# cg-tuwien/ppsurf

Measured on AMD Instinct MI355X. Metric: occupancy query-points/sec @ res=257, 50NN, higher is better.
Workload: dtype f16x3

## Files before the change

### ppsurf_amd/csrc/pps_common.h

```cpp
#pragma once
#include <hip/hip_runtime.h>
#include <stdint.h>

typedef float f32x4 __attribute__((ext_vector_type(4)));

#define PPS_WAVE 64
#define PPS_OK 0
#define PPS_ERR_ARG 1
#define PPS_ERR_LAUNCH 2

#define PPS_SG_MFMA 0x008
#define PPS_SG_DSREAD 0x100
#define PPS_SG_VALU 0x002

namespace pps {

__device__ __forceinline__ int lane_id() { return threadIdx.x & 63; }

template <int CTRL>
__device__ __forceinline__ float dpp_mov(float v) {
    return __builtin_bit_cast(float, __builtin_amdgcn_update_dpp(0, __builtin_bit_cast(int, v), CTRL, 0xf, 0xf, true));
}
__device__ __forceinline__ float row16_max(float v) {
    v = fmaxf(v, dpp_mov<0xB1>(v));
// ... 123 lines not shown
            for (int r = 0; r < 4; ++r) {
                acc0[r] = fmaxf(acc0[r], 0.f);
                acc1[r] = fmaxf(acc1[r], 0.f);
            }
        }
        out[ob] = acc0;
        out[ob + 1] = acc1;
    }
}

typedef _Float16 half8 __attribute__((ext_vector_type(8)));
typedef unsigned u32x4 __attribute__((ext_vector_type(4)));
struct HiLo { half8 hi, lo; };

__device__ __forceinline__ HiLo split_f16(const f32x4& x0, const f32x4& x1) {
    u32x4 hp, lp;
    const float v[8] = {x0.x, x0.y, x0.z, x0.w, x1.x, x1.y, x1.z, x1.w};
#pragma unroll
    for (int p = 0; p < 4; ++p) {
        const unsigned h = __builtin_bit_cast(unsigned, __builtin_amdgcn_cvt_pkrtz(v[2 * p], v[2 * p + 1]));
        unsigned l;
        asm("v_fma_mixlo_f16 %0, %1, -1.0, %2 op_sel_hi:[1,0,0]" : "=v"(l) : "v"(h), "v"(v[2 * p]));
        asm("v_fma_mixhi_f16 %0, %1, -1.0, %2 op_sel:[1,0,0] op_sel_hi:[1,0,0]" : "+v"(l) : "v"(h), "v"(v[2 * p + 1]));
        hp[p] = h;
        lp[p] = l;
    }
    return HiLo{__builtin_bit_cast(half8, hp), __builtin_bit_cast(half8, lp)};
}
#define PPS_F16_MAX 65504.f
__device__ __forceinline__ void range_track(float& amax, const f32x4& a, const f32x4& b) {
    asm volatile("v_max3_f32 %0, %0, |%1|, |%2|\n\tv_max3_f32 %0, %0, |%3|, |%4|" : "+v"(amax) : "v"(a.x), "v"(a.y), "v"(a.z), "v"(a.w));
    asm volatile("v_max3_f32 %0, %0, |%1|, |%2|\n\tv_max3_f32 %0, %0, |%3|, |%4|" : "+v"(amax) : "v"(b.x), "v"(b.y), "v"(b.z), "v"(b.w));
}
__device__ __forceinline__ HiLo split_f16_r(float& amax, const f32x4& x0, const f32x4& x1) {
    range_track(amax, x0, x1);
    return split_f16(x0, x1);
}
__device__ __forceinline__ void range_commit(float amax, int* flag) {
    if (flag != nullptr && !(amax <= PPS_F16_MAX)) atomicOr(flag, 1);
}
__device__ __forceinline__ bool gate_closed(const int* gate) { return gate != nullptr && __builtin_nontemporal_load(gate) == 0; }

__device__ __forceinline__ void join_f16(const HiLo& x, f32x4& y0, f32x4& y1) {
    const u32x4 hp = __builtin_bit_cast(u32x4, x.hi), lp = __builtin_bit_cast(u32x4, x.lo);
#pragma unroll
    for (int p = 0; p < 4; ++p) {
        float a, b;
        asm("v_fma_mix_f32 %0, %1, 1.0, %2 op_sel_hi:[1,0,1]" : "=v"(a) : "v"(hp[p]), "v"(lp[p]));
        asm("v_fma_mix_f32 %0, %1, 1.0, %2 op_sel:[1,0,1] op_sel_hi:[1,0,1]" : "=v"(b) : "v"(hp[p]), "v"(lp[p]));
        if (p < 2) { y0[2 * p] = a; y0[2 * p + 1] = b; } else { y1[2 * (p - 2)] = a; y1[2 * (p - 2) + 1] = b; }
    }
}

template <int KB, int NOB, int ACT, bool FENCE = true, bool INIT = false, class Sink, class Hook>
__device__ __forceinline__ void dense_blocks_f16x3_hook(const HiLo (&in)[KB], const half8* __restrict__ w, const f32x4* __restrict__ bias, int lane,
                                                        Sink&& sink, Hook&& hook, const f32x4* init = nullptr) {
    static_assert(NOB % 2 == 0, "output blocks are processed in pairs");
    const int g = lane >> 4;
#pragma unroll
    for (int ob = 0; ob < NOB; ob += 2) {
        f32x4 m0 = INIT ? init[ob] : bias[(ob) * 4 + g], m1 = INIT ? init[ob + 1] : bias[(ob + 1) * 4 + g];
        f32x4 c0 = {0.f, 0.f, 0.f, 0.f}, c1 = {0.f, 0.f, 0.f, 0.f};
        const half8* w0 = w + ((ob) * KB) * 128 + lane;
        const half8* w1 = w + ((ob + 1) * KB) * 128 + lane;
        half8 ph0 = w0[0], pl0 = w0[64], ph1 = w1[0], pl1 = w1[64];
#pragma unroll
        for (int kb = 0; kb < KB; ++kb) {
            const half8 ah0 = ph0, al0 = pl0, ah1 = ph1, al1 = pl1;
            if (kb + 1 < KB) {
                ph0 = w0[(kb + 1) * 128]; pl0 = w0[(kb + 1) * 128 + 64];
                ph1 = w1[(kb + 1) * 128]; pl1 = w1[(kb + 1) * 128 + 64];
            }
            m0 = __builtin_amdgcn_mfma_f32_16x16x32_f16(ah0, in[kb].hi, m0, 0, 0, 0);
            m1 = __builtin_amdgcn_mfma_f32_16x16x32_f16(ah1, in[kb].hi, m1, 0, 0, 0);
            c0 = __builtin_amdgcn_mfma_f32_16x16x32_f16(ah0, in[kb].lo, c0, 0, 0, 0);
            c1 = __builtin_amdgcn_mfma_f32_16x16x32_f16(ah1, in[kb].lo, c1, 0, 0, 0);
            c0 = __builtin_amdgcn_mfma_f32_16x16x32_f16(al0, in[kb].hi, c0, 0, 0, 0);
            c1 = __builtin_amdgcn_mfma_f32_16x16x32_f16(al1, in[kb].hi, c1, 0, 0, 0);
            hook(ob, kb);
            if (FENCE) {
                __builtin_amdgcn_sched_group_barrier(PPS_SG_DSREAD, 4, 0);
                __builtin_amdgcn_sched_group_barrier(PPS_SG_MFMA, 6, 0);
                __builtin_amdgcn_sched_barrier(0);
            }
        }
        f32x4 o0 = m0 + c0, o1 = m1 + c1;
        if (ACT == 1) {
#pragma unroll
            for (int r = 0; r < 4; ++r) { o0[r] = fmaxf(o0[r], 0.f); o1[r] = fmaxf(o1[r], 0.f); }
        }
        sink(ob >> 1, o0, o1);
    }
}
template <int KB, int NOB, int ACT, bool FENCE = true, bool INIT = false, class Sink>
__device__ __forceinline__ void dense_blocks_f16x3(const HiLo (&in)[KB], const half8* __restrict__ w, const f32x4* __restrict__ bias, int lane,
                                                   Sink&& sink, const f32x4* init = nullptr) {
    dense_blocks_f16x3_hook<KB, NOB, ACT, FENCE, INIT>(in, w, bias, lane, sink, [](int, int) {}, init);
}

template <int T, int KB, int NOB, int ACT, bool FENCE = true, class Sink>
__device__ __forceinline__ void dense_blocks_f16x3_tiles(const HiLo (&in)[T][KB], const half8* __restrict__ w, const f32x4* __restrict__ bias, int lane,
                                                         Sink&& sink) {
    static_assert(NOB % 2 == 0, "output blocks are processed in pairs");
    const int g = lane >> 4;
#pragma unroll
    for (int ob = 0; ob < NOB; ob += 2) {
        f32x4 m0[T], m1[T], c0[T], c1[T];
        const f32x4 b0 = bias[(ob) * 4 + g], b1 = bias[(ob + 1) * 4 + g];
#pragma unroll
        for (int t = 0; t < T; ++t) { m0[t] = b0; m1[t] = b1; c0[t] = f32x4{0.f, 0.f, 0.f, 0.f}; c1[t] = c0[t]; }
        const half8* w0 = w + ((ob) * KB) * 128 + lane;
        const half8* w1 = w + ((ob + 1) * KB) * 128 + lane;
        half8 ph0 = w0[0], pl0 = w0[64], ph1 = w1[0], pl1 = w1[64];
#pragma unroll
        for (int kb = 0; kb < KB; ++kb) {
            const half8 ah0 = ph0, al0 = pl0, ah1 = ph1, al1 = pl1;
            if (kb + 1 < KB) {
                ph0 = w0[(kb + 1) * 128]; pl0 = w0[(kb + 1) * 128 + 64];
                ph1 = w1[(kb + 1) * 128]; pl1 = w1[(kb + 1) * 128 + 64];
            }
#pragma unroll
            for (int t = 0; t < T; ++t) {
                m0[t] = __builtin_amdgcn_mfma_f32_16x16x32_f16(ah0, in[t][kb].hi, m0[t], 0, 0, 0);
                m1[t] = __builtin_amdgcn_mfma_f32_16x16x32_f16(ah1, in[t][kb].hi, m1[t], 0, 0, 0);
                c0[t] = __builtin_amdgcn_mfma_f32_16x16x32_f16(ah0, in[t][kb].lo, c0[t], 0, 0, 0);
                c1[t] = __builtin_amdgcn_mfma_f32_16x16x32_f16(ah1, in[t][kb].lo, c1[t], 0, 0, 0);
                c0[t] = __builtin_amdgcn_mfma_f32_16x16x32_f16(al0, in[t][kb].hi, c0[t], 0, 0, 0);
                c1[t] = __builtin_amdgcn_mfma_f32_16x16x32_f16(al1, in[t][kb].hi, c1[t], 0, 0, 0);
            }
            if (FENCE) {
                __builtin_amdgcn_sched_group_barrier(PPS_SG_DSREAD, 4, 0);
                __builtin_amdgcn_sched_group_barrier(PPS_SG_MFMA, 6 * T, 0);
                __builtin_amdgcn_sched_barrier(0);
            }
        }
#pragma unroll
        for (int t = 0; t < T; ++t) {
            f32x4 o0 = m0[t] + c0[t], o1 = m1[t] + c1[t];
            if (ACT == 1) {
#pragma unroll
                for (int r = 0; r < 4; ++r) { o0[r] = fmaxf(o0[r], 0.f); o1[r] = fmaxf(o1[r], 0.f); }
            }
            sink(t, ob >> 1, o0, o1);
        }
    }
}

template <int NOB>
__device__ __forceinline__ void xyz_blocks(float coord, f32x4* acc, const float* __restrict__ wxyz, int lane) {
#pragma unroll
// ... 51 lines not shown
```

### ppsurf_amd/csrc/pps_decode.hip

```cpp
#include <cstdlib>
#include "pps_common.h"
#include "../../include/ppsurf_amd.h"

using namespace pps;

#define NT 256
#define NW (NT / 64)
#define WG_PER_CU (512 / NT)
#ifndef PPS_PRIO
#define PPS_PRIO 1
#endif
#ifndef PPS_PRIO_PN
#define PPS_PRIO_PN 1
#endif
#define CH4 2048

template <int CHUNK_F4_NEXT, int NTH = NT, class F>
__device__ __forceinline__ void stream_step(const f32x4* __restrict__ gnext, f32x4*& cur, f32x4*& nxt, F&& compute) {
    chunk_copy_async<CHUNK_F4_NEXT / NTH, NTH>(gnext, nxt);
    compute((const f32x4*)cur);
    stream_wait();
    __syncthreads();
    f32x4* t = cur; cur = nxt; nxt = t;
}
// ... 833 lines not shown
    const int lane = lane_id(), wave = threadIdx.x >> 6, n = lane & 15, g = lane >> 4;

    lds_fill(bias_l, bias + 192, 4096);
    const f32x4* bias_g = (const f32x4*)bias;
    f32x4 *cur, *nxt;
    stream_begin<CH4>(wg, cur, nxt);
    const int ntiles = (int)((Q + NW * 16 - 1) / (NW * 16));
    int first, count, stride;
    xcd_tile_range(ntiles, first, count, stride);
    for (int it = 0; it < count; ++it) {
        const TileRow q = tile_row(first + it * stride, wave, n, Q);
        HiLo u[2];
        stn_head_h(gin + q.c * 256, wg, wg + 5 * CH4, bias_g, cur, nxt, lane, amax, u);
        half8* dst = trans2h + q.c * 1024 + g;
#pragma unroll 1
        for (int c = 0; c < 32; ++c) {
            const f32x4* gn = (c + 1 < 32) ? wg + (6 + c) * CH4 : wg;
            stream_step<CH4>(gn, cur, nxt, [&](const f32x4* w) {
                dense_blocks_f16x3<2, 8, 0, false>(u, (const half8*)w, bias4 + 32 * c, lane, [&](int i, const f32x4& o0, const f32x4& o1) {
                    const int a = 2 * c + (i >> 1), kb = i & 1;
                    const HiLo v = split_f16_r(amax, o0, o1);
                    if (q.valid) {
                        half8* d = dst + (((a >> 4) * 2 + kb) * 2) * 64 + 4 * (a & 15);
                        d[0] = v.hi;
                        d[64] = v.lo;
                    }
                }); });
        }
    }
    range_commit(amax, range);
}

#define PC_W_XYZ 256
#define PC_NBIAS (576 + 256 + 4)
#define PC_WFLOATS (4096 + 8192)
#define PC_LDS_BYTES ((PC_WFLOATS + PC_W_XYZ + PC_NBIAS) * 4)

struct PhaseC {
    const f32x4 *w_c0b, *w_c2, *bias4, *u4;
    const float* xyz_l;
};
template <int NTH>
__device__ __forceinline__ PhaseC phase_c_setup(const float* __restrict__ wpack, const f32x4* __restrict__ wdense, const float* __restrict__ bias) {
    f32x4* w_l = (f32x4*)pps_smem;
    float* xyz_l = (float*)(w_l + PC_WFLOATS / 4);
    float* bias_l = xyz_l + PC_W_XYZ;
    for (int i = threadIdx.x; i < PC_WFLOATS / 4; i += NTH) w_l[i] = wdense[i];
    lds_fill(xyz_l, wpack, PC_W_XYZ);
    lds_fill(bias_l, bias, PC_NBIAS);
    const f32x4* bias4 = (const f32x4*)bias_l;
    return PhaseC{w_l, w_l + 1024, bias4, bias4 + 144, xyz_l};
}

template <bool H>
__device__ __forceinline__ void feat_rows_query(const float* __restrict__ patches, int64_t q, int P, int ntile_rows, const half8 (&th)[4][2],
                                                const half8 (&tl)[4][2], const f32x4 (&tf)[4][4], const PhaseC& pc, float s0, float& amax, int lane,
                                                float* __restrict__ xbar) {
    const int n = lane & 15, g = lane >> 4;
    const f32x4 *bias4 = pc.bias4, *u4 = pc.u4, *w_c0b = pc.w_c0b, *w_c2 = pc.w_c2;
    const float* xyz_l = pc.xyz_l;
    f32x4 acc[8];
    float mrun = -INFINITY, ssum = 0.f;
#pragma unroll
    for (int bb = 0; bb < 8; ++bb) acc[bb] = f32x4{0.f, 0.f, 0.f, 0.f};
    for (int rb = 0; rb < ntile_rows; ++rb) {
        const int rowi = rb * 16 + n;
        const bool valid = rowi < P;
        const int rowc = valid ? rowi : P - 1;
        const float coord = (g < 3) ? patches[(q * P + rowc) * 3 + g] : 0.f;
        f32x4 x0[4], y[8];
#pragma unroll
        for (int bb = 0; bb < 4; ++bb) x0[bb] = bias4[4 * bb + g];
        xyz_blocks<4>(coord, x0, xyz_l, lane);
        relu_blocks<4>(x0);
        __builtin_amdgcn_s_setprio(PPS_PRIO_PN);
        float s = 0.f;
        if (H) {
            HiLo a[2], b[2];
            a[0] = split_f16_r(amax, x0[0], x0[1]);
            a[1] = split_f16_r(amax, x0[2], x0[3]);
            dense_blocks_f16x3<2, 4, 1>(a, (const half8*)w_c0b, bias4 + 16, lane, [&](int i, const f32x4& o0, const f32x4& o1) { b[i] = split_f16_r(amax, o0, o1); });
#pragma unroll
            for (int ob = 0; ob < 4; ++ob) {
                f32x4 o = bias4[32 + 4 * ob + g], c = {0.f, 0.f, 0.f, 0.f};
#pragma unroll
                for (int kb = 0; kb < 2; ++kb) {
                    o = __builtin_amdgcn_mfma_f32_16x16x32_f16(th[ob][kb], b[kb].hi, o, 0, 0, 0);
                    c = __builtin_amdgcn_mfma_f32_16x16x32_f16(th[ob][kb], b[kb].lo, c, 0, 0, 0);
                    c = __builtin_amdgcn_mfma_f32_16x16x32_f16(tl[ob][kb], b[kb].hi, c, 0, 0, 0);
                }
                o += c;
#pragma unroll
                for (int r = 0; r < 4; ++r) x0[ob][r] = fmaxf(o[r], 0.f);
            }
            a[0] = split_f16_r(amax, x0[0], x0[1]);
            a[1] = split_f16_r(amax, x0[2], x0[3]);
            dense_blocks_f16x3<2, 8, 1>(a, (const half8*)w_c2, bias4 + 48, lane, [&](int i, const f32x4& o0, const f32x4& o1) {
                const f32x4 w0 = u4[4 * (2 * i) + g], w1 = u4[4 * (2 * i + 1) + g];
#pragma unroll
                for (int r = 0; r < 4; ++r) s += w0[r] * o0[r] + w1[r] * o1[r];
                y[2 * i] = o0;
                y[2 * i + 1] = o1;
            });
        } else {
            f32x4 x1[4];
            dense_blocks<4, 4, 1>(x0, x1, w_c0b, bias4 + 16, lane);
#pragma unroll
            for (int ob = 0; ob < 4; ++ob) {
                f32x4 o = bias4[32 + 4 * ob + g];
#pragma unroll
                for (int kb = 0; kb < 4; ++kb) {
                    o = __builtin_amdgcn_mfma_f32_16x16x4f32(tf[ob][kb].x, x1[kb].x, o, 0, 0, 0);
                    o = __builtin_amdgcn_mfma_f32_16x16x4f32(tf[ob][kb].y, x1[kb].y, o, 0, 0, 0);
                    o = __builtin_amdgcn_mfma_f32_16x16x4f32(tf[ob][kb].z, x1[kb].z, o, 0, 0, 0);
                    o = __builtin_amdgcn_mfma_f32_16x16x4f32(tf[ob][kb].w, x1[kb].w, o, 0, 0, 0);
                }
#pragma unroll
                for (int r = 0; r < 4; ++r) x0[ob][r] = fmaxf(o[r], 0.f);
            }
            dense_blocks<4, 8, 1>(x0, y, w_c2, bias4 + 48, lane);
#pragma unroll
            for (int bb = 0; bb < 8; ++bb) {
                const f32x4 w4 = u4[4 * bb + g];
#pragma unroll
                for (int r = 0; r < 4; ++r) s += w4[r] * y[bb][r];
            }
        }
        __builtin_amdgcn_s_setprio(0);
        s += __shfl_xor(s, 16);
        s += __shfl_xor(s, 32);
        s += s0;
        const float mblk = row16_max(valid ? s : -INFINITY);
        const float mnew = fmaxf(mrun, mblk);
        const float scale = __expf(mrun - mnew);
        const float en = valid ? __expf(s - mnew) : 0.f;
        mrun = mnew;
        ssum = ssum * scale + en;
#pragma unroll
        for (int bb = 0; bb < 8; ++bb)
#pragma unroll
            for (int r = 0; r < 4; ++r) acc[bb][r] = acc[bb][r] * scale + en * y[bb][r];
    }
    const float inv = 1.f / row16_sum(ssum);
    rows16_sum_transposed8(acc, lane);
    if (n < 8) ((f32x4*)(xbar + q * 128))[4 * n + g] = acc[0] * inv;
}

template <bool H>
__global__ __launch_bounds__(PNT, 2) void pointnet_feat_rows_kernel(const float* __restrict__ patches, const float* __restrict__ trans2,
                                                                    int64_t Q, int P, const float* __restrict__ wpack,
                                                                    const f32x4* __restrict__ wdense, const float* __restrict__ bias,
                                                                    float* __restrict__ xbar, int* __restrict__ flag) {
    if (!H && gate_closed(flag)) return;
    float amax = 0.f;
    const int lane = lane_id(), wave = threadIdx.x >> 6, n = lane & 15, g = lane >> 4;
    const PhaseC pc = phase_c_setup<PNT>(wpack, wdense, bias);
    __syncthreads();
    const float s0 = ((const float*)pc.bias4)[576 + 256];
    const int ntile_rows = (P + 15) / 16;

    const int ntiles = (int)((Q + PNW - 1) / PNW);
    int first, count, stride;
    xcd_tile_range(ntiles, first, count, stride);
    for (int it = 0; it < count; ++it) {
        const int64_t q = (int64_t)(first + it * stride) * PNW + wave;
        if (q >= Q) continue;
        half8 th[4][2], tl[4][2];
        f32x4 tf[4][4];
        if (H) {
            const half8* tq = (const half8*)trans2 + q * 1024 + 4 * n + g;
#pragma unroll
            for (int ob = 0; ob < 4; ++ob)
#pragma unroll
                for (int kb = 0; kb < 2; ++kb) { th[ob][kb] = tq[((ob * 2 + kb) * 2) * 64]; tl[ob][kb] = tq[((ob * 2 + kb) * 2 + 1) * 64]; }
        } else {
            const f32x4* tq = (const f32x4*)(trans2 + q * 4096);
#pragma unroll
            for (int ob = 0; ob < 4; ++ob)
#pragma unroll
                for (int kb = 0; kb < 4; ++kb) tf[ob][kb] = tq[(16 * ob + n) * 16 + 4 * kb + g];
        }
        feat_rows_query<H>(patches, q, P, ntile_rows, th, tl, tf, pc, s0, amax, lane, xbar);
    }
    if (H) range_commit(amax, flag);
}

#define PH_LDS_BYTES (2 * CH4 * 16)
__global__ __launch_bounds__(NT, 2) void pointnet_stn_head_h_kernel(const float* __restrict__ gin, int64_t Q, const f32x4* __restrict__ w16,
                                                                    const float* __restrict__ bias, half8* __restrict__ uh, int* __restrict__ range) {
    float amax = 0.f;
    const f32x4* wg = w16;
    const int lane = lane_id(), wave = threadIdx.x >> 6, n = lane & 15, g = lane >> 4;
    const f32x4* bias_g = (const f32x4*)bias;
    f32x4 *cur, *nxt;
    stream_begin<CH4>(wg, cur, nxt);
    const int ntiles = (int)((Q + NW * 16 - 1) / (NW * 16));
    int first, count, stride;
    xcd_tile_range(ntiles, first, count, stride);
    for (int it = 0; it < count; ++it) {
        const TileRow q = tile_row(first + it * stride, wave, n, Q);
        HiLo u[2];
        stn_head_h(gin + q.c * 256, wg, wg, bias_g, cur, nxt, lane, amax, u);
        if (q.valid) {
            half8* dst = uh + q.c * 16 + g;
#pragma unroll
            for (int kb = 0; kb < 2; ++kb) { dst[(2 * kb) * 4] = u[kb].hi; dst[(2 * kb + 1) * 4] = u[kb].lo; }
        }
    }
    range_commit(amax, range);
}

#define PF_NT 512
#define PF_QSTRIDE 257
#define PF_BUF (8 * PF_QSTRIDE)
#define PF_LDS_BYTES (PC_LDS_BYTES + 3 * PF_BUF * 16)
__global__ __launch_bounds__(PF_NT, 2) void pointnet_fc3_feat_rows_kernel(const float* __restrict__ patches, const half8* __restrict__ uh,
                                                                          int64_t Q, int P, const f32x4* __restrict__ wfc,
                                                                          const float* __restrict__ bias_fc, const float* __restrict__ wpack,
                                                                          const f32x4* __restrict__ wdense, const float* __restrict__ bias,
                                                                          float* __restrict__ xbar, int* __restrict__ flag) {
    float amax = 0.f;
    half8* ex = (half8*)(pps_smem + PC_LDS_BYTES);
    const int lane = lane_id(), wave = __builtin_amdgcn_readfirstlane(threadIdx.x >> 6), n = lane & 15, g = lane >> 4;
    const PhaseC pc = phase_c_setup<PF_NT>(wpack, wdense, bias);
    const float s0 = bias[576 + 256];
    const int ntile_rows = (P + 15) / 16;
    const f32x4* w3 = wfc + 5 * CH4;
    const f32x4* b3 = (const f32x4*)(bias_fc + 192);
    half8* ex_w = ex + (n < 8 ? n * PF_QSTRIDE : PF_BUF + (n - 8) * PF_QSTRIDE) + 8 * wave + g;
    const half8* ex_r = ex + wave * PF_QSTRIDE + 4 * n + g;
    const half8* ex_r2 = ex_r + PF_BUF;

    const int ntiles = (int)((Q + 15) / 16);
    int first, count, stride;
    xcd_tile_range(ntiles, first, count, stride);
    const f32x4 tf[4][4] = {};
    for (int it = 0; it < count; ++it) {
        const int64_t q0 = (int64_t)(first + it * stride) * 16;
        half8 th[4][2], tl[4][2], th2[2][2], tl2[2][2];
        {
            const int64_t qc = q0 + n < Q ? q0 + n : Q - 1;
            HiLo u[2];
#pragma unroll
            for (int kb = 0; kb < 2; ++kb) { u[kb].hi = uh[qc * 16 + (2 * kb) * 4 + g]; u[kb].lo = uh[qc * 16 + (2 * kb + 1) * 4 + g]; }
#pragma unroll
            for (int ob = 0; ob < 4; ++ob) {
                __syncthreads();
                const int c = 8 * ob + wave;
                const half8* wc = (const half8*)(w3 + c * CH4);
                asm volatile("" : "+s"(wc));
                dense_blocks_f16x3<2, 8, 0, false>(u, wc, b3 + 32 * c, lane, [&](int i, const f32x4& o0, const f32x4& o1) {
                    const HiLo v = split_f16_r(amax, o0, o1);
                    half8* d = ex_w + (n >= 8 ? (ob & 1) * PF_BUF : 0) + ((i & 1) * 2) * 64 + 4 * (i >> 1);
                    d[0] = v.hi;
                    d[64] = v.lo;
                });
                __syncthreads();
#pragma unroll
                for (int kb = 0; kb < 2; ++kb) {
                    th[ob][kb] = ex_r[(2 * kb) * 64];
                    tl[ob][kb] = ex_r[(2 * kb + 1) * 64];
                    if (ob < 2) {
                        th2[ob][kb] = ex_r2[ob * PF_BUF + (2 * kb) * 64];
                        tl2[ob][kb] = ex_r2[ob * PF_BUF + (2 * kb + 1) * 64];
                    }
                }
            }
        }
        if (q0 + wave < Q) feat_rows_query<true>(patches, q0 + wave, P, ntile_rows, th, tl, tf, pc, s0, amax, lane, xbar);
        if (q0 + wave + 8 < Q) {
#pragma unroll
            for (int kb = 0; kb < 2; ++kb) {
#pragma unroll
                for (int ob = 0; ob < 2; ++ob) {
                    th[ob][kb] = th2[ob][kb];
                    tl[ob][kb] = tl2[ob][kb];
                    th[2 + ob][kb] = ex_r2[ob * PF_BUF + (2 * kb) * 64];
                    tl[2 + ob][kb] = ex_r2[ob * PF_BUF + (2 * kb + 1) * 64];
                }
            }
            feat_rows_query<true>(patches, q0 + wave + 8, P, ntile_rows, th, tl, tf, pc, s0, amax, lane, xbar);
        }
    }
    range_commit(amax, flag);
}

#define TL_NBIAS (256 + 256 + 32)
#define TL_LDS_BYTES (2 * CH4 * 16 + TL_NBIAS * 4)

__global__ __launch_bounds__(NT, 2) void decode_tail_kernel(const float* __restrict__ pooled, const float* __restrict__ xbar, int64_t Q,
                                                            const float* __restrict__ wpack, const float* __restrict__ bias,
                                                            float* __restrict__ logits, float* __restrict__ occ, int* __restrict__ gate) {
    if (gate_closed(gate)) return;
    if (gate != nullptr && blockIdx.x == 0 && threadIdx.x == 0) atomicAdd(gate + 1, 1);
    float* bias_l = (float*)((f32x4*)pps_smem + 2 * CH4);
    const f32x4* bias4 = (const f32x4*)bias_l;
    const f32x4* wg = (const f32x4*)wpack;
    const int lane = lane_id(), wave = threadIdx.x >> 6, n = lane & 15, g = lane >> 4;

    lds_fill(bias_l, bias, TL_NBIAS);
    f32x4 *cur, *nxt;
    stream_begin<CH4>(wg, cur, nxt);

    const int ntiles = (int)((Q + NW * 16 - 1) / (NW * 16));
    int first, count, stride;
    xcd_tile_range(ntiles, first, count, stride);
    for (int it = 0; it < count; ++it) {
        const TileRow q = tile_row(first + it * stride, wave, n, Q);
        f32x4 p[16], x[8], h[16];
        {
            const f32x4* sp = (const f32x4*)(pooled + q.c * 256) + g;
            const f32x4* sx = (const f32x4*)(xbar + q.c * 128) + g;
#pragma unroll
            for (int bb = 0; bb < 16; ++bb) p[bb] = sp[4 * bb];
#pragma unroll
            for (int bb = 0; bb < 8; ++bb) x[bb] = sx[4 * bb];
        }
#pragma unroll
        for (int c = 0; c < 8; ++c)
            stream_step<CH4>(wg + (c + 1) * CH4, cur, nxt,
                           [&](const f32x4* w) { dense_blocks<16, 2, 0>(p, &h[2 * c], w, bias4 + 8 * c, lane); });
#pragma unroll
        for (int c = 0; c < 4; ++c)
            stream_step<CH4>(wg + (c + 9) * CH4, cur, nxt,
                           [&](const f32x4* w) { dense_blocks<8, 4, 1, 1>(x, &h[4 * c], w, bias4, lane); });
#pragma unroll
        for (int c = 0; c < 8; ++c)
            stream_step<CH4>(wg + (c + 13) * CH4, cur, nxt,
                           [&](const f32x4* w) { dense_blocks<16, 2, 1>(h, &p[2 * c], w, bias4 + 64 + 8 * c, lane); });
        f32x4 o[2];
        stream_step<CH4>(wg, cur, nxt, [&](const f32x4* w) { dense_blocks<16, 2, 0>(p, o, w, bias4 + 128, lane); });
        store_logits(o[0], q, g, logits, occ);
    }
}
// ... 183 lines not shown
    if (q == 0) return PPS_OK;
    if (!G || !pts || !query || !idx || !wpack || !w16 || !bias || !wtail || !out || !guard) return PPS_ERR_ARG;
    const int grid = grid_for(q, chip_wgs(8));
    if (hipMemsetAsync(guard, 0, sizeof(int), (hipStream_t)stream) != hipSuccess) return PPS_ERR_LAUNCH;
    const float* wh = (const float*)w16;
    int rc;
    if (c == 32) {
        rc = launch<interp_small_kernel<2, true>>(grid, IS_NT, 0, stream, G, pts, query, idx, q, k, wpack, wh, bias, wtail, nout, out, guard);
        if (rc == PPS_OK) rc = launch<interp_small_kernel<2, false>>(grid, IS_NT, 0, stream, G, pts, query, idx, q, k, wpack, nullptr, bias, wtail, nout, out, guard);
    } else {
        rc = launch<interp_small_kernel<4, true>>(grid, IS_NT, 0, stream, G, pts, query, idx, q, k, wpack, wh, bias, wtail, nout, out, guard);
        if (rc == PPS_OK) rc = launch<interp_small_kernel<4, false>>(grid, IS_NT, 0, stream, G, pts, query, idx, q, k, wpack, nullptr, bias, wtail, nout, out, guard);
    }
    return rc;
}

int pps_pointnet_stn_rows_f32(const float* patches, int64_t q, int p, const float* wpack, const float* bias, float* g,
                              void* stream) {
    if (q < 0 || p < 1) return PPS_ERR_ARG;
    if (q == 0) return PPS_OK;
    if (!patches || !wpack || !bias || !g) return PPS_ERR_ARG;
    return launch_stn_rows<false>(patches, q, p, wpack, wpack + PA_W_XYZ, bias, g, nullptr, stream);
}

int pps_pointnet_stn_fc_f32(const float* g, int64_t q, const float* wpack, const float* bias, float* trans2, void* stream) {
    return stn_fc_f32_impl(g, q, wpack, bias, trans2, nullptr, stream);
}

int pps_pointnet_feat_rows_f32(const float* patches, const float* trans2, int64_t q, int p, const float* wpack,
                               const float* bias, float* xbar, void* stream) {
    if (q < 0 || p < 1) return PPS_ERR_ARG;
    if (q == 0) return PPS_OK;
    if (!patches || !trans2 || !wpack || !bias || !xbar) return PPS_ERR_ARG;
    return launch_feat_rows<false>(patches, trans2, q, p, wpack, wpack + PC_W_XYZ, bias, xbar, nullptr, stream);
}

int pps_pointnet_f16x3(const float* patches, int64_t q, int p, const float* const* weights ,
                       const void* const* w16, float* g, float* trans2, float* xbar, int32_t* range_flag, void* const* events, void* stream) {
    if (q < 0 || p < 1) return PPS_ERR_ARG;
    if (q == 0) return PPS_OK;
    if (!patches || !weights || !w16 || !w16[0] || !w16[1] || !w16[2] || !g || !trans2 || !xbar) return PPS_ERR_ARG;
    int* range = (int*)range_flag;
    auto mark = [&](int i) { if (events && events[i]) hipEventRecord((hipEvent_t)events[i], (hipStream_t)stream); };
    int rc = launch_stn_rows<true>(patches, q, p, weights[0], w16[0], weights[1], g, range, stream);
    mark(0);
    if (rc != PPS_OK) return rc;
    const int head_grid = grid_for((q + NW * 16 - 1) / (NW * 16));
    const char* fused_env = getenv("PPS_PN_FUSED");
    const bool fused = !(fused_env && fused_env[0] == '0' && fused_env[1] == 0);
    rc = fused ? launch<pointnet_stn_head_h_kernel>(head_grid, NT, PH_LDS_BYTES, stream, g, q, (const f32x4*)w16[1], weights[3], (half8*)trans2, range)
               : launch<pointnet_stn_fc_h_kernel>(head_grid, NT, PB_LDS_BYTES, stream, g, q, (const f32x4*)w16[1], weights[3], (half8*)trans2, range);
    mark(1);
    if (rc != PPS_OK) return rc;
    rc = fused ? launch<pointnet_fc3_feat_rows_kernel>(grid_for((q + 15) / 16, chip_wgs(1)), PF_NT, PF_LDS_BYTES, stream, patches, (const half8*)trans2,
                                                       q, p, (const f32x4*)w16[1], weights[3], weights[4], (const f32x4*)w16[2], weights[5], xbar, range)
               : launch_feat_rows<true>(patches, trans2, q, p, weights[4], w16[2], weights[5], xbar, range, stream);
    mark(2);
    return rc;
}

int pps_decode_tail_f32(const float* pooled, const float* xbar, int64_t q, const float* wpack, const float* bias,
                        float* logits, float* occ, void* stream) {
    return decode_tail_f32_impl(pooled, xbar, q, wpack, bias, logits, occ, nullptr, stream);
}

int pps_decode_tail_f16x3(const float* pooled, const float* xbar, int64_t q, const void* w16, const float* bias, float* logits, float* occ,
                          int32_t* range_flag, void* stream) {
    if (q < 0) return PPS_ERR_ARG;
    if (q == 0) return PPS_OK;
    if (!pooled || !xbar || !w16 || !bias || !logits) return PPS_ERR_ARG;
    return launch<decode_tail_h_kernel>(grid_for((q + NW * 16 - 1) / (NW * 16)), NT, TL_LDS_BYTES, stream, pooled, xbar, q, (const f32x4*)w16, bias,
                                        logits, occ, (int*)range_flag);
}

#define PPS_DECODE_WS_HEAD 64
size_t pps_decode_ws_bytes(int64_t q) { return q < 0 ? 0 : (size_t)q * (256 + 256 + 4096 + 256) * sizeof(float) + PPS_DECODE_WS_HEAD; }

static int decode_fwd(const float* table, const float* pts, const float* query, const int64_t* idx, int64_t q, int k,
                      const float* patches, int p, const float* const* weights, float* logits, float* occ, void* ws, void* const* events,
                      void* stream, const void* const* w16 = nullptr) {
    const void* interp_w16 = w16 ? w16[0] : nullptr;
    const bool pn16 = w16 && w16[1] && w16[2] && w16[3];
    if (q < 0) return PPS_ERR_ARG;
    if (q == 0) return PPS_OK;
    if (!weights || !ws || !logits) return PPS_ERR_ARG;
    for (int i = 0; i < 10; ++i)
        if (!weights[i]) return PPS_ERR_ARG;
    int* guard = (int*)ws;
    float* pooled = (float*)ws + PPS_DECODE_WS_HEAD / sizeof(float);
    float* g = pooled + q * 256;
    float* trans2 = g + q * 256;
    float* xbar = trans2 + q * 4096;
    hipStream_t st = (hipStream_t)stream;
    const bool split = interp_w16 || pn16 || (w16 && w16[4]);
    if (split && hipMemsetAsync(guard, 0, sizeof(int), st) != hipSuccess) return PPS_ERR_LAUNCH;
#define PPS_MARK(i) do { if (events && events[i] && hipEventRecord((hipEvent_t)events[i], st) != hipSuccess) return PPS_ERR_LAUNCH; } while (0)
    PPS_MARK(0);
    int rc = interp_w16 ? pps_interp_pool_f16x3(table, pts, query, idx, q, k, weights[0], interp_w16, weights[1], pooled, guard, stream)
                        : pps_interp_pool_f32(table, pts, query, idx, q, k, weights[0], weights[1], pooled, stream);
    PPS_MARK(1);
    if (pn16) {
        if (rc == PPS_OK) rc = pps_pointnet_f16x3(patches, q, p, weights + 2, w16 + 1, g, trans2, xbar, guard, events ? events + 2 : nullptr, stream);
    } else {
        if (rc == PPS_OK) rc = pps_pointnet_stn_rows_f32(patches, q, p, weights[2], weights[3], g, stream);
        PPS_MARK(2);
        if (rc == PPS_OK) rc = pps_pointnet_stn_fc_f32(g, q, weights[4], weights[5], trans2, stream);
        PPS_MARK(3);
        if (rc == PPS_OK) rc = pps_pointnet_feat_rows_f32(patches, trans2, q, p, weights[6], weights[7], xbar, stream);
// ... 37 lines not shown
```

Before: 13.21 million.

## Share partial last row tile between paired queries and prefetch fc3 weights across blocks

With P=50, each query's last 16-row tile holds only 2 valid rows. The feature-row kernel now packs the leftover rows of two queries processed by the same wave into one shared tile. It computes both transform matrices on that tile, picks per lane, and shuffles the second query's results back to it. This removes one mostly-wasted tile pass per query pair. Separately, the fc3 dense loop now prefetches weights and biases one output-block pair ahead, including across ob iterations, through a new hook/pre-buffer path in dense_blocks_f16x3_hook. The cost is extra register pressure (32 half8 prefetch buffers) and more complex control flow.

```diff
diff --git a/ppsurf_amd/csrc/pps_common.h b/ppsurf_amd/csrc/pps_common.h
--- a/ppsurf_amd/csrc/pps_common.h
+++ b/ppsurf_amd/csrc/pps_common.h
@@ -199,9 +199,10 @@
     }
 }
 
-template <int KB, int NOB, int ACT, bool FENCE = true, bool INIT = false, class Sink, class Hook>
+template <int KB, int NOB, int ACT, bool FENCE = true, bool INIT = false, int PRE = 0, class Sink, class Hook>
 __device__ __forceinline__ void dense_blocks_f16x3_hook(const HiLo (&in)[KB], const half8* __restrict__ w, const f32x4* __restrict__ bias, int lane,
-                                                        Sink&& sink, Hook&& hook, const f32x4* init = nullptr) {
+                                                        Sink&& sink, Hook&& hook, const f32x4* init = nullptr, const half8* pre = nullptr) {
+    static_assert(PRE % 2 == 0 && PRE <= NOB, "whole output-block pairs are handed over");
     static_assert(NOB % 2 == 0, "output blocks are processed in pairs");
     const int g = lane >> 4;
 #pragma unroll
@@ -210,13 +211,16 @@
         f32x4 c0 = {0.f, 0.f, 0.f, 0.f}, c1 = {0.f, 0.f, 0.f, 0.f};
         const half8* w0 = w + ((ob) * KB) * 128 + lane;
         const half8* w1 = w + ((ob + 1) * KB) * 128 + lane;
-        half8 ph0 = w0[0], pl0 = w0[64], ph1 = w1[0], pl1 = w1[64];
+        const half8* r0 = pre + (ob * KB) * 2;
+        const half8* r1 = pre + ((ob + 1) * KB) * 2;
+        const bool handed = ob < PRE;
+        half8 ph0 = handed ? r0[0] : w0[0], pl0 = handed ? r0[1] : w0[64], ph1 = handed ? r1[0] : w1[0], pl1 = handed ? r1[1] : w1[64];
 #pragma unroll
         for (int kb = 0; kb < KB; ++kb) {
             const half8 ah0 = ph0, al0 = pl0, ah1 = ph1, al1 = pl1;
             if (kb + 1 < KB) {
-                ph0 = w0[(kb + 1) * 128]; pl0 = w0[(kb + 1) * 128 + 64];
-                ph1 = w1[(kb + 1) * 128]; pl1 = w1[(kb + 1) * 128 + 64];
+                ph0 = handed ? r0[(kb + 1) * 2] : w0[(kb + 1) * 128]; pl0 = handed ? r0[(kb + 1) * 2 + 1] : w0[(kb + 1) * 128 + 64];
+                ph1 = handed ? r1[(kb + 1) * 2] : w1[(kb + 1) * 128]; pl1 = handed ? r1[(kb + 1) * 2 + 1] : w1[(kb + 1) * 128 + 64];
             }
             m0 = __builtin_amdgcn_mfma_f32_16x16x32_f16(ah0, in[kb].hi, m0, 0, 0, 0);
             m1 = __builtin_amdgcn_mfma_f32_16x16x32_f16(ah1, in[kb].hi, m1, 0, 0, 0);
@@ -239,10 +243,10 @@
         sink(ob >> 1, o0, o1);
     }
 }
-template <int KB, int NOB, int ACT, bool FENCE = true, bool INIT = false, class Sink>
+template <int KB, int NOB, int ACT, bool FENCE = true, bool INIT = false, int PRE = 0, class Sink>
 __device__ __forceinline__ void dense_blocks_f16x3(const HiLo (&in)[KB], const half8* __restrict__ w, const f32x4* __restrict__ bias, int lane,
-                                                   Sink&& sink, const f32x4* init = nullptr) {
-    dense_blocks_f16x3_hook<KB, NOB, ACT, FENCE, INIT>(in, w, bias, lane, sink, [](int, int) {}, init);
+                                                   Sink&& sink, const f32x4* init = nullptr, const half8* pre = nullptr) {
+    dense_blocks_f16x3_hook<KB, NOB, ACT, FENCE, INIT, PRE>(in, w, bias, lane, sink, [](int, int) {}, init, pre);
 }
 
 template <int T, int KB, int NOB, int ACT, bool FENCE = true, class Sink>
diff --git a/ppsurf_amd/csrc/pps_decode.hip b/ppsurf_amd/csrc/pps_decode.hip
--- a/ppsurf_amd/csrc/pps_decode.hip
+++ b/ppsurf_amd/csrc/pps_decode.hip
@@ -909,98 +909,133 @@
     return PhaseC{w_l, w_l + 1024, bias4, bias4 + 144, xyz_l};
 }
 
+
+struct PoolState {
+    f32x4 acc[8];
+    float mrun, ssum;
+};
+__device__ __forceinline__ void pool_reset(PoolState& st) {
+    st.mrun = -INFINITY;
+    st.ssum = 0.f;
+#pragma unroll
+    for (int bb = 0; bb < 8; ++bb) st.acc[bb] = f32x4{0.f, 0.f, 0.f, 0.f};
+}
+__device__ __forceinline__ void pool_advance(PoolState& st, bool valid, float s, const f32x4 (&y)[8]) {
+    const float mblk = row16_max(valid ? s : -INFINITY);
+    const float mnew = fmaxf(st.mrun, mblk);
+    const float scale = __expf(st.mrun - mnew);
+    const float en = valid ? __expf(s - mnew) : 0.f;
+    st.mrun = mnew;
+    st.ssum = st.ssum * scale + en;
+#pragma unroll
+    for (int bb = 0; bb < 8; ++bb)
+#pragma unroll
+        for (int r = 0; r < 4; ++r) st.acc[bb][r] = st.acc[bb][r] * scale + en * y[bb][r];
+}
+__device__ __forceinline__ void pool_finalise(PoolState& st, int64_t q, int lane, float* __restrict__ xbar) {
+    const int n = lane & 15, g = lane >> 4;
+    const float inv = 1.f / row16_sum(st.ssum);
+    rows16_sum_transposed8(st.acc, lane);
+    if (n < 8) ((f32x4*)(xbar + q * 128))[4 * n + g] = st.acc[0] * inv;
+}
+
+__device__ __forceinline__ void matrix_blocks_f16x3(const half8 (&th)[4][2], const half8 (&tl)[4][2], const HiLo (&b)[2], const f32x4* bias4, int g,
+                                                    f32x4 (&x)[4]) {
+#pragma unroll
+    for (int ob = 0; ob < 4; ++ob) {
+        f32x4 o = bias4[32 + 4 * ob + g], c = {0.f, 0.f, 0.f, 0.f};
+#pragma unroll
+        for (int kb = 0; kb < 2; ++kb) {
+            o = __builtin_amdgcn_mfma_f32_16x16x32_f16(th[ob][kb], b[kb].hi, o, 0, 0, 0);
+            c = __builtin_amdgcn_mfma_f32_16x16x32_f16(th[ob][kb], b[kb].lo, c, 0, 0, 0);
+            c = __builtin_amdgcn_mfma_f32_16x16x32_f16(tl[ob][kb], b[kb].hi, c, 0, 0, 0);
+        }
+        x[ob] = o + c;
+    }
+}
+
+template <bool H, bool SHARE, class NextMatrix>
+__device__ __forceinline__ void feat_rows_tile(float coord, half8 (&th)[4][2], half8 (&tl)[4][2], const f32x4 (&tf)[4][4], const PhaseC& pc, float s0,
+                                               float& amax, int lane, bool second, NextMatrix&& next_matrix, f32x4 (&y)[8], float& s) {
+    static_assert(H || !SHARE, "the shared tile exists in split precision only");
+    const int g = lane >> 4;
+    const f32x4 *bias4 = pc.bias4, *u4 = pc.u4, *w_c0b = pc.w_c0b, *w_c2 = pc.w_c2;
+    f32x4 x0[4];
+#pragma unroll
+    for (int bb = 0; bb < 4; ++bb) x0[bb] = bias4[4 * bb + g];
+    xyz_blocks<4>(coord, x0, pc.xyz_l, lane);
+    relu_blocks<4>(x0);
+    __builtin_amdgcn_s_setprio(PPS_PRIO_PN);
+    s = 0.f;
+    if (H) {
+        HiLo a[2], b[2];
+        a[0] = split_f16_r(amax, x0[0], x0[1]);
+        a[1] = split_f16_r(amax, x0[2], x0[3]);
+        dense_blocks_f16x3<2, 4, 1>(a, (const half8*)w_c0b, bias4 + 16, lane, [&](int i, const f32x4& o0, const f32x4& o1) { b[i] = split_f16_r(amax, o0, o1); });
+        matrix_blocks_f16x3(th, tl, b, bias4, g, x0);
+        if (SHARE) {
+            f32x4 x1[4];
+            next_matrix();
+            matrix_blocks_f16x3(th, tl, b, bias4, g, x1);
+#pragma unroll
+            for (int ob = 0; ob < 4; ++ob)
+#pragma unroll
+                for (int r = 0; r < 4; ++r) x0[ob][r] = second ? x1[ob][r] : x0[ob][r];
+        }
+        relu_blocks<4>(x0);
+        a[0] = split_f16_r(amax, x0[0], x0[1]);
+        a[1] = split_f16_r(amax, x0[2], x0[3]);
+        dense_blocks_f16x3<2, 8, 1>(a, (const half8*)w_c2, bias4 + 48, lane, [&](int i, const f32x4& o0, const f32x4& o1) {
+            const f32x4 w0 = u4[4 * (2 * i) + g], w1 = u4[4 * (2 * i + 1) + g];
+#pragma unroll
+            for (int r = 0; r < 4; ++r) s += w0[r] * o0[r] + w1[r] * o1[r];
+            y[2 * i] = o0;
+            y[2 * i + 1] = o1;
+        });
+    } else {
+        f32x4 x1[4];
+        dense_blocks<4, 4, 1>(x0, x1, w_c0b, bias4 + 16, lane);
+#pragma unroll
+        for (int ob = 0; ob < 4; ++ob) {
+            f32x4 o = bias4[32 + 4 * ob + g];
+#pragma unroll
+            for (int kb = 0; kb < 4; ++kb) {
+                o = __builtin_amdgcn_mfma_f32_16x16x4f32(tf[ob][kb].x, x1[kb].x, o, 0, 0, 0);
+                o = __builtin_amdgcn_mfma_f32_16x16x4f32(tf[ob][kb].y, x1[kb].y, o, 0, 0, 0);
+                o = __builtin_amdgcn_mfma_f32_16x16x4f32(tf[ob][kb].z, x1[kb].z, o, 0, 0, 0);
+                o = __builtin_amdgcn_mfma_f32_16x16x4f32(tf[ob][kb].w, x1[kb].w, o, 0, 0, 0);
+            }
+#pragma unroll
+            for (int r = 0; r < 4; ++r) x0[ob][r] = fmaxf(o[r], 0.f);
+        }
+        dense_blocks<4, 8, 1>(x0, y, w_c2, bias4 + 48, lane);
+#pragma unroll
+        for (int bb = 0; bb < 8; ++bb) {
+            const f32x4 w4 = u4[4 * bb + g];
+#pragma unroll
+            for (int r = 0; r < 4; ++r) s += w4[r] * y[bb][r];
+        }
+    }
+    __builtin_amdgcn_s_setprio(0);
+    s += __shfl_xor(s, 16);
+    s += __shfl_xor(s, 32);
+    s += s0;
+}
+
 template <bool H>
-__device__ __forceinline__ void feat_rows_query(const float* __restrict__ patches, int64_t q, int P, int ntile_rows, const half8 (&th)[4][2],
-                                                const half8 (&tl)[4][2], const f32x4 (&tf)[4][4], const PhaseC& pc, float s0, float& amax, int lane,
-                                                float* __restrict__ xbar) {
+__device__ __forceinline__ void feat_rows_tiles(const float* __restrict__ patches, int64_t q, int P, int ntiles, half8 (&th)[4][2], half8 (&tl)[4][2],
+                                                const f32x4 (&tf)[4][4], const PhaseC& pc, float s0, float& amax, int lane, PoolState& st) {
     const int n = lane & 15, g = lane >> 4;
-    const f32x4 *bias4 = pc.bias4, *u4 = pc.u4, *w_c0b = pc.w_c0b, *w_c2 = pc.w_c2;
-    const float* xyz_l = pc.xyz_l;
-    f32x4 acc[8];
-    float mrun = -INFINITY, ssum = 0.f;
-#pragma unroll
-    for (int bb = 0; bb < 8; ++bb) acc[bb] = f32x4{0.f, 0.f, 0.f, 0.f};
-    for (int rb = 0; rb < ntile_rows; ++rb) {
+    for (int rb = 0; rb < ntiles; ++rb) {
         const int rowi = rb * 16 + n;
         const bool valid = rowi < P;
         const int rowc = valid ? rowi : P - 1;
         const float coord = (g < 3) ? patches[(q * P + rowc) * 3 + g] : 0.f;
-        f32x4 x0[4], y[8];
-#pragma unroll
-        for (int bb = 0; bb < 4; ++bb) x0[bb] = bias4[4 * bb + g];
-        xyz_blocks<4>(coord, x0, xyz_l, lane);
-        relu_blocks<4>(x0);
-        __builtin_amdgcn_s_setprio(PPS_PRIO_PN);
-        float s = 0.f;
-        if (H) {
-            HiLo a[2], b[2];
-            a[0] = split_f16_r(amax, x0[0], x0[1]);
-            a[1] = split_f16_r(amax, x0[2], x0[3]);
-            dense_blocks_f16x3<2, 4, 1>(a, (const half8*)w_c0b, bias4 + 16, lane, [&](int i, const f32x4& o0, const f32x4& o1) { b[i] = split_f16_r(amax, o0, o1); });
-#pragma unroll
-            for (int ob = 0; ob < 4; ++ob) {
-                f32x4 o = bias4[32 + 4 * ob + g], c = {0.f, 0.f, 0.f, 0.f};
-#pragma unroll
-                for (int kb = 0; kb < 2; ++kb) {
-                    o = __builtin_amdgcn_mfma_f32_16x16x32_f16(th[ob][kb], b[kb].hi, o, 0, 0, 0);
-                    c = __builtin_amdgcn_mfma_f32_16x16x32_f16(th[ob][kb], b[kb].lo, c, 0, 0, 0);
-                    c = __builtin_amdgcn_mfma_f32_16x16x32_f16(tl[ob][kb], b[kb].hi, c, 0, 0, 0);
-                }
-                o += c;
-#pragma unroll
-                for (int r = 0; r < 4; ++r) x0[ob][r] = fmaxf(o[r], 0.f);
-            }
-            a[0] = split_f16_r(amax, x0[0], x0[1]);
-            a[1] = split_f16_r(amax, x0[2], x0[3]);
-            dense_blocks_f16x3<2, 8, 1>(a, (const half8*)w_c2, bias4 + 48, lane, [&](int i, const f32x4& o0, const f32x4& o1) {
-                const f32x4 w0 = u4[4 * (2 * i) + g], w1 = u4[4 * (2 * i + 1) + g];
-#pragma unroll
-                for (int r = 0; r < 4; ++r) s += w0[r] * o0[r] + w1[r] * o1[r];
-                y[2 * i] = o0;
-                y[2 * i + 1] = o1;
-            });
-        } else {
-            f32x4 x1[4];
-            dense_blocks<4, 4, 1>(x0, x1, w_c0b, bias4 + 16, lane);
-#pragma unroll
-            for (int ob = 0; ob < 4; ++ob) {
-                f32x4 o = bias4[32 + 4 * ob + g];
-#pragma unroll
-                for (int kb = 0; kb < 4; ++kb) {
-                    o = __builtin_amdgcn_mfma_f32_16x16x4f32(tf[ob][kb].x, x1[kb].x, o, 0, 0, 0);
-                    o = __builtin_amdgcn_mfma_f32_16x16x4f32(tf[ob][kb].y, x1[kb].y, o, 0, 0, 0);
-                    o = __builtin_amdgcn_mfma_f32_16x16x4f32(tf[ob][kb].z, x1[kb].z, o, 0, 0, 0);
-                    o = __builtin_amdgcn_mfma_f32_16x16x4f32(tf[ob][kb].w, x1[kb].w, o, 0, 0, 0);
-                }
-#pragma unroll
-                for (int r = 0; r < 4; ++r) x0[ob][r] = fmaxf(o[r], 0.f);
-            }
-            dense_blocks<4, 8, 1>(x0, y, w_c2, bias4 + 48, lane);
-#pragma unroll
-            for (int bb = 0; bb < 8; ++bb) {
-                const f32x4 w4 = u4[4 * bb + g];
-#pragma unroll
-                for (int r = 0; r < 4; ++r) s += w4[r] * y[bb][r];
-            }
-        }
-        __builtin_amdgcn_s_setprio(0);
-        s += __shfl_xor(s, 16);
-        s += __shfl_xor(s, 32);
-        s += s0;
-        const float mblk = row16_max(valid ? s : -INFINITY);
-        const float mnew = fmaxf(mrun, mblk);
-        const float scale = __expf(mrun - mnew);
-        const float en = valid ? __expf(s - mnew) : 0.f;
-        mrun = mnew;
-        ssum = ssum * scale + en;
-#pragma unroll
-        for (int bb = 0; bb < 8; ++bb)
-#pragma unroll
-            for (int r = 0; r < 4; ++r) acc[bb][r] = acc[bb][r] * scale + en * y[bb][r];
-    }
-    const float inv = 1.f / row16_sum(ssum);
-    rows16_sum_transposed8(acc, lane);
-    if (n < 8) ((f32x4*)(xbar + q * 128))[4 * n + g] = acc[0] * inv;
+        f32x4 y[8];
+        float s;
+        feat_rows_tile<H, false>(coord, th, tl, tf, pc, s0, amax, lane, false, [] {}, y, s);
+        pool_advance(st, valid, s, y);
+    }
 }
 
 template <bool H>
@@ -1037,7 +1072,10 @@
 #pragma unroll
                 for (int kb = 0; kb < 4; ++kb) tf[ob][kb] = tq[(16 * ob + n) * 16 + 4 * kb + g];
         }
-        feat_rows_query<H>(patches, q, P, ntile_rows, th, tl, tf, pc, s0, amax, lane, xbar);
+        PoolState st;
+        pool_reset(st);
+        feat_rows_tiles<H>(patches, q, P, ntile_rows, th, tl, tf, pc, s0, amax, lane, st);
+        pool_finalise(st, q, lane, xbar);
     }
     if (H) range_commit(amax, flag);
 }
@@ -1071,13 +1109,18 @@
 #define PF_QSTRIDE 257
 #define PF_BUF (8 * PF_QSTRIDE)
 #define PF_LDS_BYTES (PC_LDS_BYTES + 3 * PF_BUF * 16)
+#ifndef PF_LOOK
+#define PF_LOOK 1
+#endif
 __global__ __launch_bounds__(PF_NT, 2) void pointnet_fc3_feat_rows_kernel(const float* __restrict__ patches, const half8* __restrict__ uh,
                                                                           int64_t Q, int P, const f32x4* __restrict__ wfc,
                                                                           const float* __restrict__ bias_fc, const float* __restrict__ wpack,
                                                                           const f32x4* __restrict__ wdense, const float* __restrict__ bias,
-                                                                          float* __restrict__ xbar, int* __restrict__ flag) {
+                                                                          float* __restrict__ xbar, int* __restrict__ flag, int shared_tile) {
     float amax = 0.f;
     half8* ex = (half8*)(pps_smem + PC_LDS_BYTES);
+    const int fb = P >> 4, lo = P & 15;
+    const bool share_ok = shared_tile != 0 && fb >= 1 && lo != 0 && 2 * lo <= 16;
     const int lane = lane_id(), wave = __builtin_amdgcn_readfirstlane(threadIdx.x >> 6), n = lane & 15, g = lane >> 4;
     const PhaseC pc = phase_c_setup<PF_NT>(wpack, wdense, bias);
     const float s0 = bias[576 + 256];
@@ -1100,18 +1143,44 @@
             HiLo u[2];
 #pragma unroll
             for (int kb = 0; kb < 2; ++kb) { u[kb].hi = uh[qc * 16 + (2 * kb) * 4 + g]; u[kb].lo = uh[qc * 16 + (2 * kb + 1) * 4 + g]; }
+            half8 ahead[32];
+            f32x4 bahead[8];
+            auto request = [&](unsigned off, int t, int kb) {
+                const half8* wn = (const half8*)((const char*)w3 + off) + lane;
+#pragma unroll
+                for (int o = 0; o < 2; ++o)
+#pragma unroll
+                    for (int part = 0; part < 2; ++part) {
+                        const int j = ((2 * t + o) * 2 + kb) * 2 + part;
+                        ahead[j] = wn[64 * j];
+                    }
+                if (kb == 0) {
+                    const f32x4* bn = (const f32x4*)((const char*)b3 + (off >> 6)) + g;
+                    bahead[2 * t] = bn[4 * (2 * t)];
+                    bahead[2 * t + 1] = bn[4 * (2 * t + 1)];
+                }
+            };
+            {
+                unsigned off = (unsigned)wave * (CH4 * 16u);
+                asm volatile("" : "+s"(off));
+#pragma unroll
+                for (int t = 0; t < PF_LOOK; ++t) { request(off, t, 0); request(off, t, 1); }
+            }
 #pragma unroll
             for (int ob = 0; ob < 4; ++ob) {
                 __syncthreads();
-                const int c = 8 * ob + wave;
-                const half8* wc = (const half8*)(w3 + c * CH4);
-                asm volatile("" : "+s"(wc));
-                dense_blocks_f16x3<2, 8, 0, false>(u, wc, b3 + 32 * c, lane, [&](int i, const f32x4& o0, const f32x4& o1) {
+                unsigned coff = (unsigned)(8 * ob + wave) * (CH4 * 16u), noff = coff + 8 * (CH4 * 16u);
+                asm volatile("" : "+s"(coff), "+s"(noff));
+                dense_blocks_f16x3_hook<2, 8, 0, false, true, 8>(u, nullptr, nullptr, lane, [&](int i, const f32x4& o0, const f32x4& o1) {
                     const HiLo v = split_f16_r(amax, o0, o1);
                     half8* d = ex_w + (n >= 8 ? (ob & 1) * PF_BUF : 0) + ((i & 1) * 2) * 64 + 4 * (i >> 1);
                     d[0] = v.hi;
                     d[64] = v.lo;
-                });
+                }, [&](int b, int kb) {
+                    const int t = (b >> 1) + PF_LOOK;
+                    if (t < 4) request(coff, t, kb);
+                    else if (ob < 3) request(noff, t - 4, kb);
+                }, bahead, ahead);
                 __syncthreads();
 #pragma unroll
                 for (int kb = 0; kb < 2; ++kb) {
@@ -1124,8 +1193,9 @@
                 }
             }
         }
-        if (q0 + wave < Q) feat_rows_query<true>(patches, q0 + wave, P, ntile_rows, th, tl, tf, pc, s0, amax, lane, xbar);
-        if (q0 + wave + 8 < Q) {
+        const int64_t qa = q0 + wave, qb = qa + 8;
+        const bool share = share_ok && qb < Q;
+        auto second_matrix = [&] {
 #pragma unroll
             for (int kb = 0; kb < 2; ++kb) {
 #pragma unroll
@@ -1136,7 +1206,44 @@
                     tl[2 + ob][kb] = ex_r2[ob * PF_BUF + (2 * kb + 1) * 64];
                 }
             }
-            feat_rows_query<true>(patches, q0 + wave + 8, P, ntile_rows, th, tl, tf, pc, s0, amax, lane, xbar);
+        };
+        float sb = 0.f;
+        if (qa < Q) {
+            PoolState st;
+            pool_reset(st);
+            feat_rows_tiles<true>(patches, qa, P, share ? fb : ntile_rows, th, tl, tf, pc, s0, amax, lane, st);
+            if (share) {
+                const bool second = n >= lo && n < 2 * lo;
+                const int64_t row = second ? qb * P + 16 * fb + (n - lo) : qa * P + (n < lo ? 16 * fb + n : P - 1);
+                const float coord = (g < 3) ? patches[row * 3 + g] : 0.f;
+                f32x4 y[8];
+                float s;
+                feat_rows_tile<true, true>(coord, th, tl, tf, pc, s0, amax, lane, second, second_matrix, y, s);
+                pool_advance(st, n < lo, s, y);
+                const int from = (lane & ~15) | ((n + lo) & 15);
+#pragma unroll
+                for (int bb = 0; bb < 8; ++bb) {
+                    f32x4 v;
+#pragma unroll
+                    for (int r = 0; r < 4; ++r) v[r] = __shfl(y[bb][r], from);
+                    (bb < 4 ? th2 : tl2)[(bb >> 1) & 1][bb & 1] = __builtin_bit_cast(half8, v);
+                }
+                sb = __shfl(s, from);
+            }
+            pool_finalise(st, qa, lane, xbar);
+        }
+        if (qb < Q) {
+            PoolState st;
+            pool_reset(st);
+            if (!share) second_matrix();
+            feat_rows_tiles<true>(patches, qb, P, share ? fb : ntile_rows, th, tl, tf, pc, s0, amax, lane, st);
+            if (share) {
+                f32x4 y[8];
+#pragma unroll
+                for (int bb = 0; bb < 8; ++bb) y[bb] = __builtin_bit_cast(f32x4, (bb < 4 ? th2 : tl2)[(bb >> 1) & 1][bb & 1]);
+                pool_advance(st, n < lo, sb, y);
+            }
+            pool_finalise(st, qb, lane, xbar);
         }
     }
     range_commit(amax, flag);
@@ -1426,8 +1533,11 @@
                : launch<pointnet_stn_fc_h_kernel>(head_grid, NT, PB_LDS_BYTES, stream, g, q, (const f32x4*)w16[1], weights[3], (half8*)trans2, range);
     mark(1);
     if (rc != PPS_OK) return rc;
+    const char* share_env = getenv("PPS_FEAT_SHARED_TILE");
+    const int shared_tile = !(share_env && share_env[0] == '0' && share_env[1] == 0);
     rc = fused ? launch<pointnet_fc3_feat_rows_kernel>(grid_for((q + 15) / 16, chip_wgs(1)), PF_NT, PF_LDS_BYTES, stream, patches, (const half8*)trans2,
-                                                       q, p, (const f32x4*)w16[1], weights[3], weights[4], (const f32x4*)w16[2], weights[5], xbar, range)
+                                                       q, p, (const f32x4*)w16[1], weights[3], weights[4], (const f32x4*)w16[2], weights[5], xbar, range,
+                                                       shared_tile)
                : launch_feat_rows<true>(patches, trans2, q, p, weights[4], w16[2], weights[5], xbar, range, stream);
     mark(2);
     return rc;
```

Result: no change. 13.33 million, median of 6 (+0.9%).
